# willSapgreen/stereo-vision

Hardware: AMD Instinct MI355X
Metric: stereo pairs/sec (ELAS 1242x375, ROBOTICS, D1+D2+LR) (higher is better)
Workload: dtype u8

## Files before the change

### stereo-vision_amd/csrc/elas_engine.cpp

```cpp
#include <hip/hip_runtime.h>
#include <stdio.h>
#include <string.h>

#include <atomic>
#include <chrono>
#include <condition_variable>
#include <deque>
#include <functional>
#include <algorithm>
#include <map>
#include <memory>
#include <mutex>
#include <string>
#include <thread>
#include <vector>

#include "hip_guard.h"
#include "svh_internal.h"

namespace svh {

static thread_local int t_device = 0;

#define HIP_TRY(kind, expr) SVH_HIP_TRY(nullptr, kind, expr)
// ... 85 lines not shown
    size_t prior_cap = 0;
    size_t ntri_max = 0;
    std::vector<HostPrior> hp;
    std::vector<int32_t> P;
    StageDev stg{};
    bool stage_ok = false;
    hipEvent_t stage_ev = nullptr;
    bool resident = false;
    bool force_host = false;
    float P_key[5] = {-1, -1, -1, -1, -1};
    static constexpr int kHist = 4;
    int32_t hist_sup[kHist] = {}, hist_tri[kHist] = {};
    int hist_n = 0, hist_at = 0;
    int32_t hist_g = 0;
    svh_elas_params hist_p{};
    PhaseBSize sized{};
    size_t o_P = 0, o_sup = 0, o_tri = 0;

    void release() {
        if (!stream) return;
        (void)hipSetDevice(device);
        static_cast<LaneBufs&>(*this) = LaneBufs();
        stage_ok = false; stg = StageDev{};
        P_key[0] = -1;
        hist_n = 0;
        W = H = 0;
    }

    void destroy() {
        if (!stream) return;
        (void)hipSetDevice(device);
        release();
        for (hipEvent_t* e : {&wait_ev, &match_ev, &copy_ev, &stage_ev})
            if (*e) {
                (void)hipEventDestroy(*e);
                *e = nullptr;
            }
        for (hipEvent_t e : prof.ev) (void)hipEventDestroy(e);
        prof.ev.clear();
        prof.names.clear();
        if (copy_stream) (void)hipStreamDestroy(copy_stream);
        (void)hipStreamDestroy(stream);
        copy_stream = stream = nullptr;
    }

    int ensure(const svh_elas_params& p, int32_t w, int32_t h, int32_t g) {
        if (!stream) {
            HIP_TRY(none, hipSetDevice(device));
            HIP_TRY(none, hipStreamCreateWithFlags(&stream, hipStreamNonBlocking));
        }
        const int32_t st = p.candidate_stepsize + (p.subsampling ? p.candidate_stepsize % 2 : 0);
        if (w == W && h == H && p.disp_max == disp_max && st == step && p.grid_size == grid_size &&
            p.subsampling == sub && g <= gcap)
            return SVH_OK;
        hipStream_t keep = stream;
        release();
        stream = keep;
        d = make_dims(p, w, h);
        const size_t N = (size_t)w * h, DN = (size_t)d.DW * d.DH, G2 = (size_t)2 * g;
        LANE_GROW(img, G2 * N);
        LANE_GROW(desc, G2 * N * 16);
        LANE_GROW(owner, G2 * N * sizeof(int32_t));
        HIP_TRY(copy, hipMemset(owner, 0, G2 * N * sizeof(int32_t)));
        owner_hi = svh::env("SVH_TEST_OWNER_HI") ? atoll(svh::env("SVH_TEST_OWNER_HI")) : 0;
        LANE_GROW(Draw, G2 * DN * sizeof(float));
        LANE_GROW(D, G2 * DN * sizeof(float));
        LANE_GROW(tmp, G2 * DN * sizeof(float));
        LANE_GROW(labels, G2 * DN * sizeof(int32_t));
        LANE_GROW(counts, G2 * DN * sizeof(int32_t));
        LANE_GROW(seg_nroots, G2 * (size_t)((d.DW + 63) / 64) * ((d.DH + 15) / 16) * sizeof(int32_t));
        const size_t nc = (size_t)d.Wc * d.Hc;
        LANE_GROW(dcan, g * nc * sizeof(int16_t));
        LANE_GROW(h_dcan, g * nc * sizeof(int16_t));
        LANE_GROW(h_img, G2 * N);
        const size_t nsup = nc + 6;
        ntri_max = 2 * nsup + 8;
        prior_cap = sizeof(GroupHdr) + (size_t)(p.disp_max + 1) * sizeof(int32_t) + 512 +
                    (size_t)g * (nsup * 3 + 2 * ntri_max * 3) * sizeof(int32_t);
        LANE_GROW(prior_dev, prior_cap);
        LANE_GROW(h_prior, prior_cap);
        LANE_GROW(raster, G2 * ntri_max * sizeof(TriRaster));
        LANE_GROW(planes, G2 * ntri_max * 6 * sizeof(float));
        const size_t gw_bytes = G2 * d.gw * d.gh * d.gwords * sizeof(uint32_t);
        LANE_GROW(seed, gw_bytes);
        LANE_GROW(mask, gw_bytes);
        if (d.gwords <= 8) LANE_GROW(lists, G2 * d.gw * d.gh * 32 * sizeof(uint16_t));
        hp.resize(g);
        o_P = (sizeof(GroupHdr) + 63) & ~(size_t)63;
        o_sup = (o_P + (size_t)(p.disp_max + 1) * sizeof(int32_t) + 63) & ~(size_t)63;
        o_tri = (o_sup + (size_t)g * nsup * 3 * sizeof(int32_t) + 63) & ~(size_t)63;
        if (stage_device_ok(p, d) && o_tri + (size_t)g * 2 * ntri_max * 3 * sizeof(int32_t) <= prior_cap) {
            const size_t cap = std::min<size_t>(nsup, 65535), rec = 2 * cap + 2, S2 = (size_t)2 * g;
            size_t off = 0;
            auto take = [&](size_t bytes) { size_t at = off; off = (off + bytes + 255) & ~(size_t)255; return at; };
            const size_t a_sup = take((size_t)g * 3 * cap * 4), a_cnt = take(sizeof(StageCounts));
            const size_t a_ids = take(S2 * 4 * rec * 4), a_xys = take(S2 * 4 * rec * 4), a_nbr = take(S2 * 4 * rec * 4);
            size_t a_arr[11];
            for (int k = 0; k < 11; k++) a_arr[k] = take(S2 * cap * 4);
            const size_t a_fl = take(S2 * 2 * cap * 4), a_fr = take(S2 * 2 * cap * 4);
            const size_t a_wl = take((size_t)g * 3 * nc * 4), a_cw = take((size_t)g * (nc / 4 + 1) * 4);
            LANE_GROW(stage_blob, off);
            HIP_TRY(copy, hipMemset(stage_blob, 0, off));
            LANE_GROW(h_counts, sizeof(StageCounts));
            uint8_t* b = stage_blob;
            stg.dcan = dcan;
            stg.sup_raw = reinterpret_cast<int32_t*>(b + a_sup);
            stg.counts = reinterpret_cast<StageCounts*>(b + a_cnt);
            stg.ids = reinterpret_cast<int32_t*>(b + a_ids);
            stg.xys = reinterpret_cast<int32_t*>(b + a_xys);
            stg.nbr = reinterpret_cast<uint32_t*>(b + a_nbr);
            int32_t** ia[6] = {&stg.pxy, &stg.buck, &stg.buck2, &stg.byx, &stg.order, &stg.oxy};
            uint32_t** ua[4] = {&stg.lx, &stg.ly, &stg.tmp, &stg.P};
            for (int k = 0; k < 6; k++) *ia[k] = reinterpret_cast<int32_t*>(b + a_arr[k]);
            for (int k = 0; k < 4; k++) *ua[k] = reinterpret_cast<uint32_t*>(b + a_arr[6 + k]);
            stg.dmap = reinterpret_cast<int32_t*>(b + a_arr[10]);
            stg.fl = reinterpret_cast<uint32_t*>(b + a_fl);
            stg.fr = reinterpret_cast<uint32_t*>(b + a_fr);
            stg.wl = reinterpret_cast<int32_t*>(b + a_wl);
            stg.cntw = reinterpret_cast<uint32_t*>(b + a_cw);
            stg.sup_cap = (int32_t)cap;
            stg.rec_cap = (int32_t)rec;
            stage_ok = true;
        }
        HIP_TRY(wait, hipDeviceSynchronize());
        W = w; H = h; disp_max = p.disp_max; step = st; grid_size = p.grid_size; sub = p.subsampling;
        gcap = g;
        return SVH_OK;
    }
};

static std::atomic<int> g_wait_us{40};
static std::atomic<bool> g_hostprof{false};
static hipError_t lane_wait(Lane& L) {
    if (!L.poll_wait || g_wait_us <= 0) return hipStreamSynchronize(L.stream);
    if (!L.wait_ev) {
        hipError_t e = hipEventCreateWithFlags(&L.wait_ev, hipEventDisableTiming);
        if (e != hipSuccess) return e;
    }
    hipError_t e = hipEventRecord(L.wait_ev, L.stream);
    if (e != hipSuccess) return e;
    for (;;) {
        e = hipEventQuery(L.wait_ev);
        if (e != hipErrorNotReady) return e;
        std::this_thread::sleep_for(std::chrono::microseconds(g_wait_us.load(std::memory_order_relaxed)));
    }
}

struct Pool {
    std::mutex mu;
    std::condition_variable cv;
    std::vector<Lane*> lanes;
    std::vector<Lane*> free_list;
    int max_lanes = 4;
};

static std::mutex g_mu;

static std::map<int, Pool*>& g_pools = *new std::map<int, Pool*>();
static std::atomic<int> g_lanes{6};
static std::atomic<int> g_group{32};
static std::atomic<bool> g_group_set{false};
static std::atomic<int> g_stage_mode{-1};
static int stage_mode_from_env();
static void apply_config(const svh_config& c, int explicit_call) {
    if (explicit_call) {
        if (c.elas_workers > 0) svh_elas_set_lanes(c.elas_workers);
        if (c.elas_pairs_per_launch > 0) svh_elas_set_group(c.elas_pairs_per_launch);
// ... 405 lines not shown
                for (int k = 0; k < 2 && pinned; k++) {
                    hipPointerAttribute_t at;
                    pinned = hipPointerGetAttributes(&at, io.hI[k][j]) == hipSuccess && at.type == hipMemoryTypeHost;
                }
            (void)hipGetLastError();
            if (pinned) {
                static const bool strided_up = !(svh::env("SVH_H2D_STRIDED") && atoi(svh::env("SVH_H2D_STRIDED")) == 0);
                for (int k = 0; k < 2; k++)
                    for (int32_t j = 0; j < g;) {
                        uint8_t* dst = L.img + ((size_t)2 * j + k) * N;
                        if (io.pitch != W) {
                            HIP_TRY(copy, hipMemcpy2DAsync(dst, W, io.hI[k][j], io.pitch, W, H, hipMemcpyHostToDevice, s));
                            j++;
                            continue;
                        }
                        int32_t e = j + 1;
                        while (strided_up && e < g && io.hI[k][e] == io.hI[k][e - 1] + N) e++;
                        if (e - j > 1)
                            HIP_TRY(copy, hipMemcpy2DAsync(dst, 2 * N, io.hI[k][j], N, N, (size_t)(e - j), hipMemcpyHostToDevice, s));
                        else
                            HIP_TRY(copy, hipMemcpyAsync(dst, io.hI[k][j], N, hipMemcpyHostToDevice, s));
                        j = e;
                    }
            } else {
                for (int32_t j = 0; j < g; j++)
                    for (int k = 0; k < 2; k++) {
                        uint8_t* dst = L.h_img + ((size_t)2 * j + k) * N;
                        const uint8_t* src = io.hI[k][j];
                        if (io.pitch == W) memcpy(dst, src, N);
                        else
                            for (int32_t v = 0; v < H; v++) memcpy(dst + (size_t)v * W, src + (size_t)v * io.pitch, W);
                    }
                HIP_TRY(copy, hipMemcpyAsync(L.img, L.h_img, (size_t)2 * g * N, hipMemcpyHostToDevice, s));
            }
            img.I[0] = L.img; img.I[1] = L.img + N;
            img.stride = 2 * N; img.pitch = W;
        }
        {
            std::vector<int32_t> Pt;
            int32_t pr = 2;
            prior_table(p, Pt, &pr);
            int32_t absmax = 0;
            for (int32_t dd = 0; dd <= pr && dd < (int32_t)Pt.size(); dd++)
                absmax = std::max(absmax, (int32_t)std::min<int64_t>(std::llabs((long long)Pt[dd]), INT32_MAX));
            static const int fly_env = svh::env("SVH_DESC_FLY") ? atoi(svh::env("SVH_DESC_FLY")) : 1;
            L.desc_fly = (!tapping || fly_env == 2) && descriptors_on_the_fly(p, d, absmax, pr, L.lists != nullptr);
        }
        if (tapping && L.desc_fly) {
            launch_descriptor(cx, img, g, W, H, p.subsampling, L.desc, false);
            int rc2 = tap_dev(L, taps, SVH_ELAS_DESC1, L.desc.p, N * 16); if (rc2) return rc2;
            rc2 = tap_dev(L, taps, SVH_ELAS_DESC2, L.desc.p + N * 16, N * 16); if (rc2) return rc2;
            HIP_TRY(wait, hipStreamSynchronize(s));
        }
        launch_descriptor(cx, img, g, W, H, p.subsampling, L.desc, L.desc_fly);
        launch_support(cx, p, d, g, L.desc, L.dcan, L.desc_fly);
        const int sm = g_stage_mode.load();
        L.resident = !L.force_host && L.stage_ok &&
                     (sm == 1 || (sm < 0 && prefer_device && stage_device_preferred(p, d, prefer_device > 1)));
        if (L.resident && prefer_device) L.poll_wait = true;
        if (!L.resident || tapping)
            HIP_TRY(copy, hipMemcpyAsync(L.h_dcan, L.dcan, g * nc * sizeof(int16_t), hipMemcpyDeviceToHost, s));
        if (L.resident) {
            prior_table(p, L.P, &plane_radius);
            const float key[5] = {p.beta, p.gamma, p.sigma, p.sradius, (float)p.disp_max};
            if (memcmp(key, L.P_key, sizeof(key)) != 0) {
                memcpy(L.h_prior + L.o_P, L.P.data(), L.P.size() * sizeof(int32_t));
                HIP_TRY(copy, hipMemcpyAsync(L.prior_dev + L.o_P, L.h_prior + L.o_P, L.P.size() * sizeof(int32_t),
                                       hipMemcpyHostToDevice, s));
                HIP_TRY(wait, hipStreamSynchronize(s));
                memcpy(L.P_key, key, sizeof(key));
            }
            if (tapping) {
                HIP_TRY(wait, hipStreamSynchronize(s));
                if (!L.desc_fly) {
                    rc = tap_dev(L, taps, SVH_ELAS_DESC1, L.desc.p, N * 16); if (rc) return rc;
                    rc = tap_dev(L, taps, SVH_ELAS_DESC2, L.desc.p + N * 16, N * 16); if (rc) return rc;
                }
                tap_host(taps, SVH_ELAS_DCAN_RAW, L.h_dcan.p, nc);
            }
            const bool blits = svh::env("SVH_STAGE_BLITS") && atoi(svh::env("SVH_STAGE_BLITS")) != 0;
            launch_stage_device(cx, p, d, g, L.stg, reinterpret_cast<GroupHdr*>(L.prior_dev.p),
                                reinterpret_cast<int32_t*>(L.prior_dev + L.o_sup),
                                reinterpret_cast<int32_t*>(L.prior_dev + L.o_tri),
                                blits ? nullptr : L.seed.p, (size_t)2 * g * d.gw * d.gh * d.gwords,
                                blits ? nullptr : L.h_counts.p);
            if (!L.stage_ev) HIP_TRY(none, hipEventCreateWithFlags(&L.stage_ev, hipEventDisableTiming));
            if (blits) HIP_TRY(copy, hipMemcpyAsync(L.h_counts, L.stg.counts, sizeof(StageCounts), hipMemcpyDeviceToHost, s));
            HIP_TRY(none, hipEventRecord(L.stage_ev, s));
            if (tapping) {
                HIP_TRY(copy, hipMemcpyAsync(hdr, L.prior_dev, sizeof(GroupHdr), hipMemcpyDeviceToHost, s));
                HIP_TRY(wait, hipStreamSynchronize(s));
                if (hdr->active[0]) {
                    rc = tap_dev(L, taps, SVH_ELAS_SUPPORT, reinterpret_cast<int32_t*>(L.prior_dev + L.o_sup),
                                 (size_t)3 * hdr->total_sup); if (rc) return rc;
                    rc = tap_dev(L, taps, SVH_ELAS_TRI1, reinterpret_cast<int32_t*>(L.prior_dev + L.o_tri),
                                 (size_t)3 * hdr->tri_end[0]); if (rc) return rc;
                    rc = tap_dev(L, taps, SVH_ELAS_TRI2,
                                 reinterpret_cast<int32_t*>(L.prior_dev + L.o_tri) + (size_t)3 * hdr->tri_end[0],
                                 (size_t)3 * (hdr->tri_end[1] - hdr->tri_end[0])); if (rc) return rc;
                }
            }
            L.sized = PhaseBSize{};
            if (!tapping || hdr->active[0]) {
                const int32_t tri_bound = 2 * g * 2 * L.stg.sup_cap;
                int32_t hint_sup = 0, hint_tri = 0;
                const bool use_hist = !(svh::env("SVH_PHASEB_HISTORY") && atoi(svh::env("SVH_PHASEB_HISTORY")) == 0);
                if (use_hist && L.hist_n && L.hist_g == g && memcmp(&L.hist_p, &p, sizeof(p)) == 0)
                    for (int k = 0; k < L.hist_n; k++) {
                        hint_sup = std::max(hint_sup, L.hist_sup[k]);
                        hint_tri = std::max(hint_tri, L.hist_tri[k]);
                    }
                L.sized = phase_b_size(d, g, -1, -1, hint_sup, hint_tri);
                L.sized.seed_cleared = !blits;
                rc = enqueue_phase_b(L.o_P, L.o_sup, L.o_tri, -1, -1, tri_bound, L.sized);
                if (rc) return rc;
            }
        }
        HP_MARK(HP_ENQ_A);
    }
    if (!(mode & RG_HOST_B)) return SVH_OK;
    double t1 = t0, t2 = t0;
    if (L.resident) {
        if (!io.out_device) {
            HIP_TRY(wait, event_wait(L, L.stage_ev));
            HP_MARK(HP_WAIT);
            int32_t active[kMaxGroup];
            for (int32_t j = 0; j < g; j++) active[j] = active_of(j);
            rc = copy_out(active);
            if (rc) return rc;
        }
        if (g_hostprof) g_hp_pairs += g;
        HP_MARK(HP_ENQ_B);
        t1 = t2 = now_ms();
    } else {
    const bool warm = L.parallel_host && g == 1;
    if (warm) helpers_warm(3, 1500);
    struct WarmOff {
        bool on;
        ~WarmOff() { if (on) helpers_warm(0, 0); }
    } warm_off{warm};
    HIP_TRY(wait, lane_wait(L));
    HIP_TRY(launch, hipGetLastError());
    L.prof.collect();
    HP_MARK(HP_WAIT);
    if (g_hostprof) g_hp_pairs += g;
    t1 = now_ms();
    if (tapping) {
        if (!L.desc_fly) {
            rc = tap_dev(L, taps, SVH_ELAS_DESC1, L.desc.p, N * 16); if (rc) return rc;
            rc = tap_dev(L, taps, SVH_ELAS_DESC2, L.desc.p + N * 16, N * 16); if (rc) return rc;
        }
        tap_host(taps, SVH_ELAS_DCAN_RAW, L.h_dcan.p, nc);
    }

    memset(hdr, 0, sizeof(GroupHdr));
    hdr->npairs = g;
    int32_t total_sup = 0, total_tri = 0, nactive = 0;
    for (int32_t j = 0; j < g; j++) {
        HostPrior& hp = L.hp[j];
        support_from_candidates(p, d, L.h_dcan + j * nc, hp.support, false);
        HP_MARK(HP_FILTER);
        hdr->sup_off[j] = total_sup;
        status[j] = SVH_OK;
        if (hp.support.size() / 3 < 3) {
            printf("ERROR: Need at least 3 support points!\n");
            fflush(stdout);
            status[j] = SVH_ERR_FEW_SUPPORT;
// ... 834 lines not shown
```

### stereo-vision_amd/csrc/elas_kernels.hip

```cpp
#include <hip/hip_runtime.h>

#include <algorithm>
#include <cstdlib>

#include "dev_common.h"
#include "prior_core.h"
#include "svh_internal.h"

namespace svh {

namespace {

constexpr int kWave = 64;

template <int kCtrl, int kRowMask>
__device__ __forceinline__ uint32_t dpp_min_step(uint32_t v) {
    const uint32_t o =
        (uint32_t)__builtin_amdgcn_update_dpp((int)0xFFFFFFFFu, (int)v, kCtrl, kRowMask, 0xF, false);
    return o < v ? o : v;
}

__device__ __forceinline__ uint32_t wave_min_u32(uint32_t v) {
    v = dpp_min_step<0xB1, 0xF>(v);
    v = dpp_min_step<0x4E, 0xF>(v);
// ... 557 lines not shown
            const int x0 = rgt ? xr0 : xl0, x1 = rgt ? xr1 : xl1, w = rgt ? wrs : wls;
            uint4* dst = (rgt ? sR : sL) + row * w - x0;
#pragma unroll
            for (int i = 0; i < 4; i++)
                if (x + i >= x0 && x + i <= x1) dst[x + i] = o[i];
        }
        for (int task = (int)threadIdx.x; task < nr + kSB; task += kST) {
            if (task < nr) {
                const int x = ar0 + 4 * task;
                uint4 o[4];
                fly_desc4_off(pl1, imstride + (uint32_t)v * fpitch + 8u + (uint32_t)x, fpitch, vplane, o);
                if (x == 0 || x + 4 > P.W - 3) {
#pragma unroll
                    for (int i = 0; i < 4; i++)
                        if (x + i < 3 || x + i >= P.W - 3) o[i] = make_uint4(0, 0, 0, 0);
                }
#pragma unroll
                for (int i = 0; i < 4; i++)
                    if (x + i >= xr0 && x + i <= xr1) s_texR[x + i - xr0] = (uint16_t)texture16(o[i]);
            } else {
                const int c = task - nr, u = (uc0 + c) * P.step;
                s_texL[c] = (uint16_t)(c < ncand && u < P.W ? texture16(fly_desc1(pl1, P.W, P.H, u, v)) : 0u);
            }
        }
    } else {
    stage_slots<6>(s_strip, 2 * (wls + wrs), (int)threadIdx.x, kST, [&](int i) {
        const bool rgt = i >= 2 * wls;
        const int j = rgt ? i - 2 * wls : i, w = rgt ? wrs : wls, wreal = rgt ? wr : wl;
        const int row = j >= w, xx = j - row * w, x = xx < wreal ? xx : wreal - 1;
        return (rgt ? d2 : d1)[(size_t)(v + (row ? 2 : -2)) * P.W + (rgt ? xr0 : xl0) + x];
    });
    }
    __syncthreads();
    const StripView L = {sL, xl0, wls}, R = {sR, xr0, wrs};
    constexpr int kNW = kST / kWave, kPerRound = 4 * kNW;
    static_assert(kSB % kPerRound == 0 && kSB <= 256, "whole rounds; candidate indices fit a byte");
    const int grp = lane >> 4;
    const int gl = lane & 15;
    __shared__ int16_t s_fwd[kSB];
    __shared__ uint8_t s_todo[kSB];
    __shared__ int s_ntodo;
#pragma unroll
    for (int rep = 0; rep < kSB / kPerRound; rep++) {
        const int c = rep * kPerRound + wave + grp * kNW;
        if (rep * kPerRound >= ncand) break;
        const bool have = c < ncand;
        const int uc = uc0 + (have ? c : 0), u = uc * P.step;
        const bool in = have && uc > 0 && u >= 5 && u <= P.W - 6;
        const int t1 = !in ? 0 : kFly ? (int)s_texL[c] : (int)texture16(d1[(size_t)v * P.W + u]);
        const int d = support_match_rows(L, R, t1, u, false, in, P, gl);
        if (gl == 0 && c < kSB) s_fwd[c] = (int16_t)(have ? d : -1);
    }
    __syncthreads();
    if (wave == 0) {
        int base = 0;
#pragma unroll
        for (int c0 = 0; c0 < kSB; c0 += kWave) {
            const int c = c0 + lane;
            const int mine = c < ncand ? (int)s_fwd[c] : -1;
            const uint64_t mask = __builtin_amdgcn_ballot_w64(mine >= 0);
            if (mine >= 0) s_todo[base + __builtin_popcountll(mask & ((1ull << lane) - 1))] = (uint8_t)c;
            base += __builtin_popcountll(mask);
            if (c < ncand && mine < 0) dcan[c] = (int16_t)((uc0 + c) > 0 ? -1 : 0);
        }
        if (lane == 0) s_ntodo = base;
    }
    __syncthreads();
    const int ntodo = s_ntodo;
    for (int t0 = 4 * wave; t0 < ntodo; t0 += kPerRound) {
        const int t = t0 + grp;
        const bool have = t < ntodo;
        const int c = have ? (int)s_todo[t] : 0;
        const int d = have ? (int)s_fwd[c] : 0;
        const int uc = uc0 + c, u = uc * P.step;
        const int ub = have ? u - d : 5;
        const int t2 = !have ? 0 : kFly ? (int)s_texR[ub - xr0] : (int)texture16(d2[(size_t)v * P.W + ub]);
        const int dd = support_match_rows(R, L, t2, ub, true, have, P, gl);
        const int diff = d > dd ? d - dd : dd - d;
        const int out = (dd >= 0 && diff <= P.lr_threshold) ? d : -1;
        if (have && gl == 0) dcan[c] = (int16_t)out;
    }
}

__global__ __launch_bounds__(256) void k_prior(GroupDev G, int total_tri_arg) {
    const int total_tri = total_tri_arg >= 0 ? total_tri_arg : G.hdr->total_tri;
    for (int gid = blockIdx.x * 256 + threadIdx.x; (gid - (int)threadIdx.x) < 2 * total_tri; gid += gridDim.x * 256) {
    const int T = gid >> 1, rs = gid & 1;
    const bool live = T < total_tri;
    const int Tc = live ? T : 0;
    int first;
    const int slot = tri_slot(G.hdr, Tc, &first);
    const int pair = slot >> 1, side = slot & 1;
    const int32_t* sup = G.support + 3 * (size_t)G.hdr->sup_off[pair];
    const int32_t* c = G.tri + 3 * (size_t)Tc;
    int32_t su[3], sv[3], sd[3];
#pragma unroll
    for (int k = 0; k < 3; k++) {
        const int32_t* s = sup + 3 * c[k];
        su[k] = s[0];
        sv[k] = s[1];
        sd[k] = s[2];
    }
    float mine[3];
    {
        double A[3][3], B[3];
#pragma unroll
        for (int r = 0; r < 3; r++) {
            A[r][0] = (double)(rs ? su[r] - sd[r] : su[r]);
            A[r][1] = (double)sv[r];
            A[r][2] = 1.0;
            B[r] = (double)sd[r];
        }
        if (prior::solve3(A, B)) {
            mine[0] = (float)B[0];
            mine[1] = (float)B[1];
            mine[2] = (float)B[2];
        } else {
            mine[0] = mine[1] = mine[2] = 0.f;
        }
    }
    float pl[6];
#pragma unroll
    for (int k = 0; k < 3; k++) {
        const float other = __shfl_xor(mine[k], 1);
        pl[k] = rs ? other : mine[k];
        pl[3 + k] = rs ? mine[k] : other;
    }
    if (!live || rs) continue;
#pragma unroll
    for (int k = 0; k < 6; k++) G.planes[6 * (size_t)T + k] = pl[k];

    float tu[3], tv[3];
#pragma unroll
    for (int k = 0; k < 3; k++) {
        tu[k] = side ? (float)(su[k] - sd[k]) : (float)su[k];
        tv[k] = (float)sv[k];
    }
#pragma unroll
    for (int j = 0; j < 3; j++)
#pragma unroll
        for (int k = 0; k < j; k++)
            if (tu[k] > tu[j]) {
                float a = tu[j]; tu[j] = tu[k]; tu[k] = a;
                float b = tv[j]; tv[j] = tv[k]; tv[k] = b;
            }
    TriRaster r;
    const float Au = tu[0], Av = tv[0], Bu = tu[1], Bv = tv[1], Cu = tu[2], Cv = tv[2];
    r.uA = (int32_t)Au;
    r.uB = (int32_t)Bu;
    r.uC = (int32_t)Cu;
    float ABa = 0.f, ACa = 0.f, BCa = 0.f;
    if (r.uA != r.uB) ABa = __fdiv_rn(__fsub_rn(Av, Bv), __fsub_rn(Au, Bu));
    if (r.uA != r.uC) ACa = __fdiv_rn(__fsub_rn(Av, Cv), __fsub_rn(Au, Cu));
    if (r.uB != r.uC) BCa = __fdiv_rn(__fsub_rn(Bv, Cv), __fsub_rn(Bu, Cu));
    r.ABa = ABa;
    r.ACa = ACa;
    r.BCa = BCa;
    r.ABb = __fsub_rn(Av, __fmul_rn(ABa, Au));
    r.ACb = __fsub_rn(Av, __fmul_rn(ACa, Au));
    r.BCb = __fsub_rn(Bv, __fmul_rn(BCa, Bu));
    const float pa = side ? pl[3] : pl[0];
    const float pd = side ? pl[0] : pl[3];
    r.pa = pa;
    r.pb = side ? pl[4] : pl[1];
    r.pc = side ? pl[5] : pl[2];
    r.valid = ((double)fabsf(pa) < 0.7 && (double)fabsf(pd) < 0.7) ? 1 : 0;
    r.slot = slot;
    r.first = first;
    r.pad_[0] = 0;
    G.raster[T] = r;
    }
}

__global__ __launch_bounds__(256) void k_grid_seed(GroupDev G, int total_sup_arg, int gw, int gh,
                                                   int gwords, int grid_size, int disp_max) {
    const int total_sup = total_sup_arg >= 0 ? total_sup_arg : G.hdr->total_sup;
    for (int S = blockIdx.x * 256 + threadIdx.x; S < total_sup; S += gridDim.x * 256) {
    int pair = 0;
    while (pair < G.hdr->npairs - 1 && S >= G.hdr->sup_off[pair + 1]) pair++;
    const int32_t* s = G.support + 3 * (size_t)S;
    const int xc = s[0], yc = s[1], dc = s[2];
    const int y = (int)floorf(__fdiv_rn((float)yc, (float)grid_size));
    const int xl = (int)floorf((float)(xc / grid_size));
    const int xr = (int)floorf(__fdiv_rn((float)(xc - dc), (float)grid_size));
    const int lo = dc - 1 > 0 ? dc - 1 : 0, hi = dc + 1 < disp_max ? dc + 1 : disp_max;
    const size_t cells = (size_t)gw * gh;
#pragma unroll
    for (int side = 0; side < 2; side++) {
        const int x = side ? xr : xl;
        if (x < 0 || x >= gw || y < 0 || y >= gh) continue;
        uint32_t* cell = G.seed + (((size_t)(2 * pair + side) * cells) + (size_t)y * gw + x) * gwords;
        for (int dd = lo; dd <= hi; dd++) atomicOr(&cell[dd >> 5], 1u << (dd & 31));
    }
    }
}

__global__ __launch_bounds__(256) void k_grid_dilate(GroupDev G, int slots, int gw, int gh,
                                                     int gwords) {
    const int i = blockIdx.x * 256 + threadIdx.x;
    const int cells = gw * gh;
    const int per = cells * gwords;
    if (i >= slots * per) return;
    const int z = i / per, rem = i - z * per;
    const int c = rem / gwords, w = rem - c * gwords;
    uint32_t o = 0;
    if (c >= gw + 1 && c <= cells - gw - 2) {
        const uint32_t* base = G.seed + (size_t)z * per + w;
        const int nb[9] = {-gw - 1, -gw, -gw + 1, -1, 0, 1, gw - 1, gw, gw + 1};
#pragma unroll
        for (int k = 0; k < 9; k++) o |= base[(size_t)(c + nb[k]) * gwords];
    }
    G.mask[i] = o;
}

__global__ __launch_bounds__(256) void k_grid_list(GroupDev G, int ncells, int gwords) {
    const int lane = threadIdx.x & 63;
    const int cell = __builtin_amdgcn_readfirstlane((int)((blockIdx.x * 256 + threadIdx.x) >> 6));
    if (cell >= ncells) return;
    const uint32_t* bits = G.mask + (size_t)cell * gwords;
    const uint32_t wq = lane < gwords ? bits[lane] : 0u;
    uint16_t* rec = G.lists + (size_t)cell * 32;
    int n = 0, last = 0;
#pragma unroll
    for (int q = 0; q < 4; q++) {
        const uint64_t m = (uint64_t)(uint32_t)__builtin_amdgcn_readlane((int)wq, 2 * q) |
                           ((uint64_t)(uint32_t)__builtin_amdgcn_readlane((int)wq, 2 * q + 1) << 32);
        if ((m >> lane) & 1) {
            const int idx = n + (int)__builtin_amdgcn_mbcnt_hi((uint32_t)(m >> 32), __builtin_amdgcn_mbcnt_lo((uint32_t)m, 0));
            if (idx < 28) rec[idx] = (uint16_t)((64 * q + lane) * 16);
        }
        if (m) last = 64 * q + 63 - __builtin_clzll(m);
        n += __builtin_popcountll(m);
    }
    if (lane < 31 && lane >= n) rec[lane] = (uint16_t)(last * 16);
    if (lane == 31) rec[31] = (uint16_t)n;
    if (lane >= 28 && lane < 31 && lane < n) rec[lane] = (uint16_t)(last * 16);
}

template <bool kFix>
__global__ __launch_bounds__(256) void k_owner(GroupDev G, int total_tri_arg, int W, int H, int sub, int fix_all) {
    const int total_tri = total_tri_arg >= 0 ? total_tri_arg : G.hdr->total_tri;
    const int lane = threadIdx.x & 63;
    const int need = (((total_tri + 3) >> 2) + 7) >> 3, have = (int)(gridDim.x >> 3);
    const int per_xcd = need < have ? need : have;
    if ((int)(blockIdx.x >> 3) >= per_xcd) return;
    const int bid = (int)(blockIdx.x & 7) * per_xcd + (int)(blockIdx.x >> 3);
    for (int T = __builtin_amdgcn_readfirstlane((int)((bid * 256 + threadIdx.x) >> 6)); T < total_tri;
         T += per_xcd * 32) {
    const TriRaster tr = G.raster[T];
    const int slot = tr.slot, first = tr.first;
    const int t = G.owner_base + 1 + (T - first);
    int32_t* owner = G.owner + (size_t)slot * W * H;
    const int cl = lane & 15, rp = lane >> 4;
    {
        const int ulo = tr.uA > 2 ? tr.uA : 2, uhi = tr.uC < W - 2 ? tr.uC : W - 2;
        for (int u = ulo + cl; u < uhi; u += 16) {
            if (sub && (u & 1)) continue;
            const bool second = u >= tr.uB;
            const float ea = second ? tr.BCa : tr.ABa, eb = second ? tr.BCb : tr.ABb;
            const float fu = (float)u;
            const int v1 = f2u2i(__fadd_rn(__fmul_rn(tr.ACa, fu), tr.ACb));
            const int v2 = f2u2i(__fadd_rn(__fmul_rn(ea, fu), eb));
            int va = v1 < v2 ? v1 : v2, vb = v1 < v2 ? v2 : v1;
            va = va > 0 ? va : 0;
            vb = vb < H ? vb : H;
            if (kFix && !fix_all) {
                const int v = rp < 2 ? va + rp : vb - 4 + rp;
                const bool mine = v >= va && v < vb && (rp < 2 || v >= va + 2);
                if (mine && !(sub && (v & 1))) {
                    int32_t* px = &owner[(size_t)v * W + u];
                    if (*px < t) atomicMax(px, t);
                }
            } else {
                for (int v = va + rp; v < vb; v += 4) {
                    if (sub && (v & 1)) continue;
                    int32_t* px = &owner[(size_t)v * W + u];
                    if (kFix) {
                        if (*px < t) atomicMax(px, t);
                    } else {
                        *px = t;
                    }
                }
            }
        }
    }
    }
}

struct MatchParams {
    int W, H, DW, DH, gw, gh, gwords, grid_size, sub;
    int disp_max, match_texture, plane_radius, npairs;
    uint32_t grid_magic;
};

template <bool kLds>
__global__ __launch_bounds__(kLds ? 512 : 256) void k_match(GroupDev G, MatchParams P) {
    extern __shared__ uint4 s_row[];
    __shared__ int s_P[64];
    const int z = blockIdx.z, pair = z >> 1, side = z & 1;
    if (!G.hdr->active[pair]) return;
    const int y = kLds ? blockIdx.y : blockIdx.y * 4 + threadIdx.y;
    {
        const int tl = kLds ? (int)threadIdx.x : (int)(threadIdx.y * 64 + threadIdx.x);
        if (tl < 64) s_P[tl] = tl <= P.disp_max ? G.P[tl] : 0;
    }
    const size_t N = (size_t)P.W * P.H;
    const int mul = P.sub ? 2 : 1;
    const int v = y * mul;
    int line = v < P.H - 3 ? v : P.H - 3;
    line = line > 2 ? line : 2;
    const uint4* oth_line =
        reinterpret_cast<const uint4*>(G.desc + (size_t)(z ^ 1) * N * 16) + (size_t)line * P.W;
    const int s0 = 0;
    if (kLds)
        for (int i = threadIdx.x; i < P.W; i += blockDim.x) s_row[i] = oth_line[i];
    __syncthreads();
    for (int x = kLds ? (int)threadIdx.x : (int)(blockIdx.x * 64 + threadIdx.x); x < P.DW;
         x += kLds ? (int)blockDim.x : P.DW) {
    if (y >= P.DH) return;
    const int u = x * mul;
    float out = -10.f;
    const int tri0 = z ? G.hdr->tri_end[z - 1] : 0;
    const int t = G.owner[(size_t)z * N + (size_t)v * P.W + u] - G.owner_base - 1;
    if (t >= 0 && u >= 2 && u < P.W - 2) {
        const uint4* own_line =
            reinterpret_cast<const uint4*>(G.desc + (size_t)z * N * 16) + (size_t)line * P.W;
        const uint4 own = own_line[u];
        if ((int)texture16(own) >= P.match_texture) {
            const float4 pl = *reinterpret_cast<const float4*>(G.raster + tri0 + t);
            const float pa = pl.x, pb = pl.y, pc = pl.z;
            const int valid = __float_as_int(pl.w);
            const int d_plane = (int)__fadd_rn(
                __fadd_rn(__fmul_rn(pa, (float)u), __fmul_rn(pb, (float)v)), pc);
            int dlo = d_plane - P.plane_radius;
            dlo = dlo > 0 ? dlo : 0;
            int dhi = d_plane + P.plane_radius;
            dhi = dhi < P.disp_max ? dhi : P.disp_max;
            const int cell = (v / P.grid_size) * P.gw + u / P.grid_size;
            const uint32_t* bits = G.mask + ((size_t)z * P.gw * P.gh + cell) * P.gwords;
            int min_val = 10000, min_d = -1;
            uint32_t wbuf[8];
            const bool fast8 = P.gwords == 8;
            if (fast8) {
                const uint4 lo4 = reinterpret_cast<const uint4*>(bits)[0];
                const uint4 hi4 = reinterpret_cast<const uint4*>(bits)[1];
                wbuf[0] = lo4.x; wbuf[1] = lo4.y; wbuf[2] = lo4.z; wbuf[3] = lo4.w;
                wbuf[4] = hi4.x; wbuf[5] = hi4.y; wbuf[6] = hi4.z; wbuf[7] = hi4.w;
            }
            for (int w = 0; w < P.gwords; w++) {
                uint32_t b;
                if (fast8) {
                    b = wbuf[0];
#pragma unroll
                    for (int q = 1; q < 8; q++) b = (w == q) ? wbuf[q] : b;
                } else {
                    b = bits[w];
                }
                while (b) {
                    const int dc = w * 32 + __builtin_ctz(b);
                    b &= b - 1;
                    if (dc < dlo || dc > dhi) {
                        const int uw = side ? u + dc : u - dc;
                        if (uw < 2 || uw >= P.W - 2) continue;
                        const uint4 o = kLds ? s_row[uw - s0] : oth_line[uw];
                        const int val = (int)sad16(own, o);
                        if (val < min_val) {
                            min_val = val;
                            min_d = dc;
// ... 1365 lines not shown
        if (p) p->end();
    }
};

#define LAUNCH(name, kernel, grid, block, ...)                                                  \
    do {                                                                                        \
        Timed timed_(cx, name);                                                                 \
        hipLaunchKernelGGL(kernel, grid, block, 0, (hipStream_t)cx.stream, __VA_ARGS__);        \
    } while (0)

}

void launch_descriptor(const LaunchCtx& cx, const DevImages& img, int32_t g, int32_t W, int32_t H,
                       int32_t half, uint8_t* desc, bool fly) {
    if (fly) {
        const int strips = (W + 4 * 62 - 1) / (4 * 62);
        const int cols = 4 * ((W + 4 * strips - 1) / (4 * strips));
        const int segs = (H + SP_ROWS - 1) / SP_ROWS, nwaves = strips * segs;
        LAUNCH("k_descriptor", k_sobel_planes, dim3((nwaves + 3) / 4, 2 * g), dim3(256), img, W, H, strips, cols,
               nwaves, desc);
        return;
    }
    constexpr int rows = 26, chunk = 16;
    static_assert((rows + 6) % chunk == 0, "the walk is a whole number of load chunks");
    const int strips = (W + DS_COLS - 1) / DS_COLS, segs = (H + rows - 1) / rows, nwaves = strips * segs;
    LAUNCH("k_descriptor", (k_descriptor_stream<rows, chunk>), dim3((nwaves + 3) / 4, 2 * g), dim3(256), img, W, H,
           half, strips, nwaves, desc);
}

static int support_strip(const svh_elas_params& p, const Dims& d, size_t* lds_out) {
    static const int sb_env = svh::env("SVH_SUPPORT_SB") ? atoi(svh::env("SVH_SUPPORT_SB")) : 64;
    constexpr size_t kSupportStatic = 512;
    auto strip_lds = [&](int sb) {
        const int span = (sb - 1) * d.step;
        const size_t wl = (size_t)std::min(d.W, span + 2 * p.disp_max + 5);
        const size_t wr = (size_t)std::min(d.W, span + p.disp_max + 5);
        return 2 * (size_t)(support_stride((int)wl) + support_stride((int)wr)) * sizeof(uint4);
    };
    int sb = sb_env == 32 ? 32 : 64;
    if (sb == 64 && strip_lds(64) + 2 * (size_t)d.W + 16 + kSupportStatic > 64 * 1024) sb = 32;
    const size_t lds = strip_lds(sb) + 2 * (size_t)std::min(d.W, (sb - 1) * d.step + p.disp_max + 5) + 16;
    if (lds_out) *lds_out = lds;
    return lds + kSupportStatic <= 64 * 1024 ? sb : 0;
}

void launch_support(const LaunchCtx& cx, const svh_elas_params& p, const Dims& d, int32_t g,
                    const uint8_t* desc, int16_t* dcan, bool fly) {
    SupportParams P;
    P.W = d.W; P.H = d.H; P.Wc = d.Wc; P.Hc = d.Hc; P.step = d.step; P.npairs = g;
    P.disp_min = p.disp_min; P.disp_max = p.disp_max;
    P.support_texture = p.support_texture; P.lr_threshold = p.lr_threshold;
    P.support_threshold = p.support_threshold;
    size_t lds = 0;
    const int sb = support_strip(p, d, &lds);
    if (sb) {
        Timed timed_(cx, "k_support");
        const int chunks = (d.Wc + sb - 1) / sb;
        const dim3 grid((unsigned)(((d.Hc * g + 7) / 8) * 8 * chunks), 1, 1);
        hipStream_t st = (hipStream_t)cx.stream;
        if (sb == 32 && fly) hipLaunchKernelGGL((k_support_lds<32, 512, true>), grid, dim3(512), lds, st, desc, dcan, P);
        else if (sb == 32) hipLaunchKernelGGL((k_support_lds<32, 512, false>), grid, dim3(512), lds, st, desc, dcan, P);
        else if (fly) hipLaunchKernelGGL((k_support_lds<64, 512, true>), grid, dim3(512), lds, st, desc, dcan, P);
        else hipLaunchKernelGGL((k_support_lds<64, 512, false>), grid, dim3(512), lds, st, desc, dcan, P);
    } else {
        const int cands = d.Wc * d.Hc;
        LAUNCH("k_support", k_support, dim3((cands + 3) / 4, g), dim3(256), desc, dcan, P);
    }
}

PhaseBSize phase_b_size(const Dims& d, int32_t g, int32_t total_sup, int32_t total_tri, int32_t hint_sup, int32_t hint_tri) {
    const int sup_bound = std::max(256, g * d.Wc * d.Hc / 6), tri_bound = 4 * sup_bound;
    PhaseBSize z;
    z.from_history = total_tri < 0 && total_sup < 0 && hint_sup > 0 && hint_tri > 0;
    z.ns = total_sup >= 0 ? total_sup : z.from_history ? std::min(sup_bound, hint_sup + hint_sup / 8 + 1) : sup_bound;
    z.nt = total_tri >= 0 ? total_tri : z.from_history ? std::min(tri_bound, hint_tri + hint_tri / 8 + 1) : tri_bound;
    z.seed_cleared = false;
    return z;
}

void launch_prior(const LaunchCtx& cx, const svh_elas_params& p, const Dims& d, int32_t g,
                  int32_t total_sup, int32_t total_tri, const GroupDev& G, const PhaseBSize& size) {
    hipStream_t s = (hipStream_t)cx.stream;
    const int cells = d.gw * d.gh;
    const size_t words = (size_t)2 * g * cells * d.gwords;
    if (!size.seed_cleared) (void)hipMemsetAsync(G.seed, 0, words * sizeof(uint32_t), s);
    const int nt = size.nt, ns = size.ns;
    if (nt > 0) LAUNCH("k_prior", k_prior, dim3((2 * nt + 255) / 256), dim3(256), G, total_tri);
    if (ns > 0)
        LAUNCH("k_grid_seed", k_grid_seed, dim3((ns + 255) / 256), dim3(256), G, total_sup,
               d.gw, d.gh, d.gwords, p.grid_size, p.disp_max);
    LAUNCH("k_grid_dilate", k_grid_dilate, dim3((unsigned)((words + 255) / 256)), dim3(256), G,
           2 * g, d.gw, d.gh, d.gwords);
    if (d.gwords <= 8 && G.lists)
        LAUNCH("k_grid_list", k_grid_list, dim3((unsigned)((2 * g * cells + 3) / 4)), dim3(256), G, 2 * g * cells,
               d.gwords);
}

void launch_owner(const LaunchCtx& cx, const svh_elas_params& p, const Dims& d, int32_t g,
                  int32_t total_tri, const GroupDev& G, const PhaseBSize& size) {
    if (total_tri == 0) return;
    const int nt = size.nt;
    const bool wide = (double)d.H * ((double)d.W + 2.0 * p.disp_max) > 4194304.0;
    const int fix_all = svh::env("SVH_OWNER_FIX_ALL") ? atoi(svh::env("SVH_OWNER_FIX_ALL")) : (wide ? 1 : 0);
    const dim3 go(xcd_blocks((nt + 3) / 4));
    LAUNCH("k_owner", k_owner<false>, go, dim3(256), G, total_tri, d.W, d.H,
           p.subsampling, 0);
    LAUNCH("k_owner_fix", k_owner<true>, go, dim3(256), G, total_tri, d.W, d.H,
           p.subsampling, fix_all);
}

static bool match_list_usable(const svh_elas_params& p, const Dims& d, int32_t prior_absmax, int32_t plane_radius,
                              bool have_lists, MatchList* Qout, size_t* lds_out) {
    static const bool ordered = svh::env("SVH_MATCH_ORDERED") != nullptr;
    const bool keyed_ok = !ordered && prior_absmax < (1 << 19) && p.disp_max < 512 && plane_radius <= 15 &&
                          d.W < 65536 && p.grid_size > 1;
    static const bool list_off = svh::env("SVH_MATCH_LIST") && atoi(svh::env("SVH_MATCH_LIST")) == 0;
    static const bool list_sub = !(svh::env("SVH_MATCH_LIST_SUB") && atoi(svh::env("SVH_MATCH_LIST_SUB")) == 0);
    if (!(keyed_ok && !list_off && (!p.subsampling || list_sub) && d.gwords <= 8 && have_lists && prior_absmax < 28000 &&
          d.DW <= 8 * 256))
        return false;
    MatchList Q;
    Q.Wr = (d.W + 7) / 8 * 8;
    Q.Ws = ((d.W + 3) & ~3) + 2;
    static const bool wide768 = !(svh::env("SVH_MATCH_WIDE768") && atoi(svh::env("SVH_MATCH_WIDE768")) == 0);
    int iters = (d.DW + 255) / 256;
    Q.half = std::min(256, ((d.DW + iters - 1) / iters + 63) / 64 * 64);
    if (iters > 5 && wide768 && d.DW <= 5 * 384) {
        iters = (d.DW + 383) / 384;
        Q.half = std::min(384, ((d.DW + iters - 1) / iters + 63) / 64 * 64);
    }
    Q.kIters = iters <= 5 ? 5 : 8;
    static const bool xcd_rows = !(svh::env("SVH_MATCH_XCD") && atoi(svh::env("SVH_MATCH_XCD")) == 0);
    Q.xcd = xcd_rows ? 1 : 0;
    const size_t ldsl = (size_t)2 * Q.Ws * sizeof(uint4) + (size_t)2 * d.gw * ML_CAP * sizeof(uint16_t) +
                        (size_t)2 * Q.Wr * sizeof(int16_t);
    constexpr size_t kListStatic = 256;
    bool ok = ldsl + kListStatic <= 160 * 1024;
    if (ok && ldsl + kListStatic > 64 * 1024) {
        ok = hipFuncSetAttribute((const void*)k_match_list<true, 5>, hipFuncAttributeMaxDynamicSharedMemorySize,
                                 160 * 1024 - (int)kListStatic) == hipSuccess &&
             hipFuncSetAttribute((const void*)k_match_list<false, 5>, hipFuncAttributeMaxDynamicSharedMemorySize,
                                 160 * 1024 - (int)kListStatic) == hipSuccess &&
             hipFuncSetAttribute((const void*)k_match_list<true, 8>, hipFuncAttributeMaxDynamicSharedMemorySize,
                                 160 * 1024 - (int)kListStatic) == hipSuccess &&
             hipFuncSetAttribute((const void*)k_match_list<false, 8>, hipFuncAttributeMaxDynamicSharedMemorySize,
                                 160 * 1024 - (int)kListStatic) == hipSuccess;
        if (!ok) (void)hipGetLastError();
    }
    if (Qout) *Qout = Q;
    if (lds_out) *lds_out = ldsl;
    return ok;
}

static bool match_keyed_usable(const svh_elas_params& p, const Dims& d, int32_t prior_absmax, int32_t plane_radius,
                               bool with_lr, size_t* lds2_out) {
    static const bool ordered = svh::env("SVH_MATCH_ORDERED") != nullptr;
    const bool keyed_ok = !ordered && prior_absmax < (1 << 19) && p.disp_max < 512 && plane_radius <= 15 &&
                          d.W < 65536 && p.grid_size > 1;
    const size_t lds = (size_t)d.W * sizeof(uint4);
    const size_t lds2 = 2 * lds + (with_lr ? (size_t)2 * d.DW * sizeof(float) : 0);
    if (lds2_out) *lds2_out = lds2;
    constexpr size_t keyed_lds_max = 96 * 1024;
    constexpr size_t kStaticLds = 64 * sizeof(int);
    bool use_keyed = keyed_ok && lds2 + kStaticLds <= keyed_lds_max;
    if (use_keyed && lds2 + kStaticLds > 64 * 1024) {
        use_keyed = hipFuncSetAttribute((const void*)k_match_keyed<true>, hipFuncAttributeMaxDynamicSharedMemorySize,
                                        (int)keyed_lds_max) == hipSuccess &&
                    hipFuncSetAttribute((const void*)k_match_keyed<false>, hipFuncAttributeMaxDynamicSharedMemorySize,
                                        (int)keyed_lds_max) == hipSuccess;
        if (!use_keyed) (void)hipGetLastError();
    }
    return use_keyed;
}

bool descriptors_on_the_fly(const svh_elas_params& p, const Dims& d, int32_t prior_absmax, int32_t plane_radius,
                            bool have_lists) {
    static const bool off = svh::env("SVH_DESC_FLY") && atoi(svh::env("SVH_DESC_FLY")) == 0;
    static const bool keyed_fly = !(svh::env("SVH_DESC_FLY_KEYED") && atoi(svh::env("SVH_DESC_FLY_KEYED")) == 0);
    if (off || d.W < 8 || support_strip(p, d, nullptr) == 0) return false;
    if (match_list_usable(p, d, prior_absmax, plane_radius, have_lists, nullptr, nullptr)) return true;
    return keyed_fly && match_keyed_usable(p, d, prior_absmax, plane_radius, true, nullptr);
}

bool launch_match(const LaunchCtx& cx, const svh_elas_params& p, const Dims& d, int32_t g,
                  const GroupDev& G, const DevMaps* lr_out, bool write_raw, const char** error) {
    if (error) *error = nullptr;
    MatchParams P;
    P.W = d.W; P.H = d.H; P.DW = d.DW; P.DH = d.DH; P.gw = d.gw; P.gh = d.gh; P.gwords = d.gwords;
    P.grid_size = p.grid_size; P.sub = p.subsampling; P.disp_max = p.disp_max;
    P.match_texture = p.match_texture; P.plane_radius = G.plane_radius;
    P.grid_magic = (uint32_t)(0x100000000ull / (uint64_t)p.grid_size) + 1u;
// ... 430 lines not shown
```

### stereo-vision_amd/csrc/svh_internal.h

```cpp
#ifndef SVH_INTERNAL_H
#define SVH_INTERNAL_H

#include <stddef.h>
#include <stdint.h>

#include <functional>
#include <vector>

#include "../../include/svh.h"
#include "svh_config.h"

namespace svh {

struct Dims {
    int32_t W, H;
    int32_t DW, DH;
    int32_t step;
    int32_t Wc, Hc;
    int32_t gw, gh;
    int32_t gwords;
};
Dims make_dims(const svh_elas_params& p, int32_t W, int32_t H);

constexpr int kMaxGroup = 32;
// ... 41 lines not shown
    int32_t ntri[2 * kMaxGroup];
    int32_t flags[kMaxGroup];
    int64_t dbg[32];
    int32_t dt_m[2 * kMaxGroup];
    int32_t dt_depth[2 * kMaxGroup];
};
enum { STG_DUP = 1,
       STG_OVERFLOW = 2,
       STG_FEW = 4 };
struct StageDev {
    int16_t* dcan;
    int32_t* sup_raw;
    StageCounts* counts;
    int32_t* ids;
    int32_t* xys;
    uint32_t* nbr;
    int32_t *pxy, *buck, *buck2, *byx, *order, *oxy;
    int32_t* dmap;
    uint32_t *lx, *ly, *tmp, *P;
    uint32_t *fl, *fr;
    int32_t* wl;
    uint32_t* cntw;
    int32_t sup_cap, rec_cap;
};
struct LaunchCtx;
bool stage_device_ok(const svh_elas_params& p, const Dims& d);
bool stage_device_preferred(const svh_elas_params& p, const Dims& d, bool deep_batch = false);

struct Profiler {
    virtual void begin(const char* kernel) = 0;
    virtual void end() = 0;
    virtual ~Profiler() {}
};
struct LaunchCtx {
    void* stream;
    Profiler* prof;
    bool latency = false;
};

struct DevImages {
    const uint8_t* I[2];
    size_t stride;
    int32_t pitch;
};
struct DevMaps {
    float* D[2];
    size_t stride[2];
};

struct GroupDev {
    const GroupHdr* hdr;
    const int32_t* support;
    const int32_t* tri;
    const int32_t* P;
    TriRaster* raster;
    float* planes;
    uint32_t* seed;
    uint32_t* mask;
    uint16_t* lists;
    const uint8_t* desc;
    int32_t* owner;
    float* Draw;
    int32_t plane_radius;
    int32_t owner_base;
    int32_t prior_absmax;
    int32_t desc_fly;
};

void launch_stage_device(const LaunchCtx& cx, const svh_elas_params& p, const Dims& d, int32_t g,
                         const StageDev& S, GroupHdr* hdr, int32_t* support, int32_t* tri,
                         uint32_t* seed, size_t seed_words, StageCounts* h_counts);

void launch_descriptor(const LaunchCtx& cx, const DevImages& img, int32_t g, int32_t W, int32_t H,
                       int32_t half, uint8_t* desc, bool fly);
bool descriptors_on_the_fly(const svh_elas_params& p, const Dims& d, int32_t prior_absmax, int32_t plane_radius,
                            bool have_lists);
void launch_support(const LaunchCtx& cx, const svh_elas_params& p, const Dims& d, int32_t g,
                    const uint8_t* desc, int16_t* dcan, bool fly);
struct PhaseBSize {
    int32_t ns, nt;
    bool from_history;
    bool seed_cleared;
};
PhaseBSize phase_b_size(const Dims& d, int32_t g, int32_t total_sup, int32_t total_tri, int32_t hint_sup, int32_t hint_tri);
void launch_prior(const LaunchCtx& cx, const svh_elas_params& p, const Dims& d, int32_t g,
                  int32_t total_sup, int32_t total_tri, const GroupDev& G, const PhaseBSize& size);
void launch_owner(const LaunchCtx& cx, const svh_elas_params& p, const Dims& d, int32_t g,
                  int32_t total_tri, const GroupDev& G, const PhaseBSize& size);
bool launch_match(const LaunchCtx& cx, const svh_elas_params& p, const Dims& d, int32_t g,
                  const GroupDev& G, const DevMaps* lr_out, bool write_raw, const char** error);
void launch_lr(const LaunchCtx& cx, const svh_elas_params& p, const Dims& d, int32_t g,
               const GroupDev& G, const DevMaps& out);
struct PostScratch {
    float* tmp;
    int32_t* labels;
    int32_t* counts;
    int32_t* nroots;
};
bool post_tiles_ok(const svh_elas_params& p);
void launch_gap_mean_tiles(const LaunchCtx& cx, const svh_elas_params& p, const Dims& d, int32_t g,
                           int32_t nside, const GroupDev& G, const DevMaps& out, const PostScratch& S);
void launch_segments(const LaunchCtx& cx, const svh_elas_params& p, const Dims& d, int32_t g,
                     int32_t nside, const GroupDev& G, const DevMaps& out, const PostScratch& s, bool mask = true);
void launch_gap(const LaunchCtx& cx, const svh_elas_params& p, const Dims& d, int32_t g,
                int32_t nside, const GroupDev& G, const DevMaps& out, const PostScratch& s);
void launch_adaptive_mean(const LaunchCtx& cx, const svh_elas_params& p, const Dims& d, int32_t g,
                          int32_t nside, const GroupDev& G, const DevMaps& out, const PostScratch& s);
void launch_median(const LaunchCtx& cx, const Dims& d, int32_t g, int32_t nside, const GroupDev& G,
                   const DevMaps& out, const PostScratch& s);
void launch_segments_label(const LaunchCtx& cx, const svh_elas_params& p, const Dims& d, int32_t g,
                           int32_t nside, const GroupDev& G, const DevMaps& in, const PostScratch& s);

}
#endif
```

Before: 34230.

## Replace full owner fix pass with corner-only pass guarded by per-slot validity flags

k_prior now checks whether the float edge rasterization is consistent with the integer vertices and sets a per-slot flag when it is not, and k_owner flags slots whose edge spans look inverted. The owner fix pass becomes a lighter k_owner_corner kernel that touches only the corner columns of each triangle unless its slot is flagged, in which case it walks all columns. The flags sit at the tail of the seed buffer, which is grown and cleared to hold them. This cuts the second full per-triangle column walk, at the cost of extra checks in k_prior and k_owner, and correctness now depends on the flag heuristics catching every case.

```diff
diff --git a/stereo-vision_amd/csrc/elas_engine.cpp b/stereo-vision_amd/csrc/elas_engine.cpp
--- a/stereo-vision_amd/csrc/elas_engine.cpp
+++ b/stereo-vision_amd/csrc/elas_engine.cpp
@@ -191,7 +191,7 @@
         LANE_GROW(raster, G2 * ntri_max * sizeof(TriRaster));
         LANE_GROW(planes, G2 * ntri_max * 6 * sizeof(float));
         const size_t gw_bytes = G2 * d.gw * d.gh * d.gwords * sizeof(uint32_t);
-        LANE_GROW(seed, gw_bytes);
+        LANE_GROW(seed, gw_bytes + G2 * sizeof(uint32_t));
         LANE_GROW(mask, gw_bytes);
         if (d.gwords <= 8) LANE_GROW(lists, G2 * d.gw * d.gh * 32 * sizeof(uint16_t));
         hp.resize(g);
@@ -763,7 +763,7 @@
             launch_stage_device(cx, p, d, g, L.stg, reinterpret_cast<GroupHdr*>(L.prior_dev.p),
                                 reinterpret_cast<int32_t*>(L.prior_dev + L.o_sup),
                                 reinterpret_cast<int32_t*>(L.prior_dev + L.o_tri),
-                                blits ? nullptr : L.seed.p, (size_t)2 * g * d.gw * d.gh * d.gwords,
+                                blits ? nullptr : L.seed.p, seed_words_with_flags(d, g),
                                 blits ? nullptr : L.h_counts.p);
             if (!L.stage_ev) HIP_TRY(none, hipEventCreateWithFlags(&L.stage_ev, hipEventDisableTiming));
             if (blits) HIP_TRY(copy, hipMemcpyAsync(L.h_counts, L.stg.counts, sizeof(StageCounts), hipMemcpyDeviceToHost, s));
diff --git a/stereo-vision_amd/csrc/elas_kernels.hip b/stereo-vision_amd/csrc/elas_kernels.hip
--- a/stereo-vision_amd/csrc/elas_kernels.hip
+++ b/stereo-vision_amd/csrc/elas_kernels.hip
@@ -663,7 +663,7 @@
     }
 }
 
-__global__ __launch_bounds__(256) void k_prior(GroupDev G, int total_tri_arg) {
+__global__ __launch_bounds__(256) void k_prior(GroupDev G, int total_tri_arg, uint32_t* __restrict__ oflag) {
     const int total_tri = total_tri_arg >= 0 ? total_tri_arg : G.hdr->total_tri;
     for (int gid = blockIdx.x * 256 + threadIdx.x; (gid - (int)threadIdx.x) < 2 * total_tri; gid += gridDim.x * 256) {
     const int T = gid >> 1, rs = gid & 1;
@@ -748,7 +748,31 @@
     r.valid = ((double)fabsf(pa) < 0.7 && (double)fabsf(pd) < 0.7) ? 1 : 0;
     r.slot = slot;
     r.first = first;
-    r.pad_[0] = 0;
+    {
+        const long long cr = (long long)(r.uB - r.uA) * (long long)((int)Cv - (int)Av) -
+                             (long long)((int)Bv - (int)Av) * (long long)(r.uC - r.uA);
+        const int sgn = cr > 0 ? 1 : cr < 0 ? -1 : 0;
+        r.pad_[0] = sgn;
+        bool bad = false;
+        if (r.uA < r.uC) {
+            const int iAv = (int)Av, iBv = (int)Bv;
+            const int kAC = f2u2i(__fadd_rn(__fmul_rn(r.ACa, Au), r.ACb));
+            bad = kAC != iAv && kAC != iAv - 1;
+            if (r.uA < r.uB) {
+                const int kAB = f2u2i(__fadd_rn(__fmul_rn(r.ABa, Au), r.ABb));
+                bad = bad || (kAB != iAv && kAB != iAv - 1);
+            }
+            if (r.uB < r.uC) {
+                const int kBC = f2u2i(__fadd_rn(__fmul_rn(r.BCa, Bu), r.BCb));
+                bad = bad || (kBC != iBv && kBC != iBv - 1);
+                if (r.uA < r.uB) {
+                    const int kACb = f2u2i(__fadd_rn(__fmul_rn(r.ACa, Bu), r.ACb));
+                    bad = bad || (sgn > 0 ? kACb < iBv : sgn < 0 ? kACb >= iBv : true);
+                }
+            }
+        }
+        if (bad) oflag[slot] = 1u;
+    }
     G.raster[T] = r;
     }
 }
@@ -819,7 +843,8 @@
 }
 
 template <bool kFix>
-__global__ __launch_bounds__(256) void k_owner(GroupDev G, int total_tri_arg, int W, int H, int sub, int fix_all) {
+__global__ __launch_bounds__(256) void k_owner(GroupDev G, int total_tri_arg, int W, int H, int sub, int fix_all,
+                                               uint32_t* __restrict__ oflag) {
     const int total_tri = total_tri_arg >= 0 ? total_tri_arg : G.hdr->total_tri;
     const int lane = threadIdx.x & 63;
     const int need = (((total_tri + 3) >> 2) + 7) >> 3, have = (int)(gridDim.x >> 3);
@@ -833,6 +858,7 @@
     const int t = G.owner_base + 1 + (T - first);
     int32_t* owner = G.owner + (size_t)slot * W * H;
     const int cl = lane & 15, rp = lane >> 4;
+    bool inverted = !kFix && fix_all != 0;
     {
         const int ulo = tr.uA > 2 ? tr.uA : 2, uhi = tr.uC < W - 2 ? tr.uC : W - 2;
         for (int u = ulo + cl; u < uhi; u += 16) {
@@ -845,6 +871,7 @@
             int va = v1 < v2 ? v1 : v2, vb = v1 < v2 ? v2 : v1;
             va = va > 0 ? va : 0;
             vb = vb < H ? vb : H;
+            if (!kFix) inverted = inverted || (u != tr.uA && (v1 < v2 ? tr.pad_[0] >= 0 : (v1 > v2 && tr.pad_[0] <= 0)));
             if (kFix && !fix_all) {
                 const int v = rp < 2 ? va + rp : vb - 4 + rp;
                 const bool mine = v >= va && v < vb && (rp < 2 || v >= va + 2);
@@ -865,6 +892,43 @@
             }
         }
     }
+    if (!kFix && inverted) oflag[slot] = 1u;
+    }
+}
+
+__global__ __launch_bounds__(256) void k_owner_corner(GroupDev G, int total_tri_arg, int W, int H, int sub,
+                                                      const uint32_t* __restrict__ oflag) {
+    const int total_tri = total_tri_arg >= 0 ? total_tri_arg : G.hdr->total_tri;
+    const int need = (((total_tri + 31) >> 5) + 7) >> 3, have = (int)(gridDim.x >> 3);
+    const int per_xcd = need < have ? need : have;
+    if ((int)(blockIdx.x >> 3) >= per_xcd) return;
+    const int bid = (int)(blockIdx.x & 7) * per_xcd + (int)(blockIdx.x >> 3);
+    const int col = (threadIdx.x >> 2) & 1, rp = threadIdx.x & 3;
+    for (int T = bid * 32 + (int)(threadIdx.x >> 3); T < total_tri; T += per_xcd * 256) {
+        const TriRaster tr = G.raster[T];
+        const int t = G.owner_base + 1 + (T - tr.first);
+        int32_t* owner = G.owner + (size_t)tr.slot * W * H;
+        const int ulo = tr.uA > 2 ? tr.uA : 2, uhi = tr.uC < W - 2 ? tr.uC : W - 2;
+        const bool walk = oflag[tr.slot] != 0;
+        int u = walk ? ulo + col : col ? tr.uB : tr.uA;
+        const int uend = walk ? uhi : (col && tr.uB == tr.uA) || u < ulo ? u : (u + 1 < uhi ? u + 1 : uhi);
+        for (; u < uend; u += 2) {
+            if (sub && (u & 1)) continue;
+            const bool second = u >= tr.uB;
+            const float ea = second ? tr.BCa : tr.ABa, eb = second ? tr.BCb : tr.ABb;
+            const float fu = (float)u;
+            const int v1 = f2u2i(__fadd_rn(__fmul_rn(tr.ACa, fu), tr.ACb));
+            const int v2 = f2u2i(__fadd_rn(__fmul_rn(ea, fu), eb));
+            int va = v1 < v2 ? v1 : v2, vb = v1 < v2 ? v2 : v1;
+            va = va > 0 ? va : 0;
+            vb = vb < H ? vb : H;
+            const int v = rp < 2 ? va + rp : vb - 4 + rp;
+            const bool mine = v >= va && v < vb && (rp < 2 || v >= va + 2);
+            if (mine && !(sub && (v & 1))) {
+                int32_t* px = &owner[(size_t)v * W + u];
+                if (*px < t) atomicMax(px, t);
+            }
+        }
     }
 }
 
@@ -2396,10 +2460,10 @@
                   int32_t total_sup, int32_t total_tri, const GroupDev& G, const PhaseBSize& size) {
     hipStream_t s = (hipStream_t)cx.stream;
     const int cells = d.gw * d.gh;
-    const size_t words = (size_t)2 * g * cells * d.gwords;
-    if (!size.seed_cleared) (void)hipMemsetAsync(G.seed, 0, words * sizeof(uint32_t), s);
+    const size_t words = seed_words(d, g);
+    if (!size.seed_cleared) (void)hipMemsetAsync(G.seed, 0, seed_words_with_flags(d, g) * sizeof(uint32_t), s);
     const int nt = size.nt, ns = size.ns;
-    if (nt > 0) LAUNCH("k_prior", k_prior, dim3((2 * nt + 255) / 256), dim3(256), G, total_tri);
+    if (nt > 0) LAUNCH("k_prior", k_prior, dim3((2 * nt + 255) / 256), dim3(256), G, total_tri, G.seed + words);
     if (ns > 0)
         LAUNCH("k_grid_seed", k_grid_seed, dim3((ns + 255) / 256), dim3(256), G, total_sup,
                d.gw, d.gh, d.gwords, p.grid_size, p.disp_max);
@@ -2416,11 +2480,17 @@
     const int nt = size.nt;
     const bool wide = (double)d.H * ((double)d.W + 2.0 * p.disp_max) > 4194304.0;
     const int fix_all = svh::env("SVH_OWNER_FIX_ALL") ? atoi(svh::env("SVH_OWNER_FIX_ALL")) : (wide ? 1 : 0);
+    const int force_walk = svh::env("SVH_OWNER_FORCE_WALK") && atoi(svh::env("SVH_OWNER_FORCE_WALK")) != 0 ? 1 : 0;
+    uint32_t* oflag = G.seed + seed_words(d, g);
     const dim3 go(xcd_blocks((nt + 3) / 4));
     LAUNCH("k_owner", k_owner<false>, go, dim3(256), G, total_tri, d.W, d.H,
-           p.subsampling, 0);
-    LAUNCH("k_owner_fix", k_owner<true>, go, dim3(256), G, total_tri, d.W, d.H,
-           p.subsampling, fix_all);
+           p.subsampling, force_walk, oflag);
+    if (fix_all == 0)
+        LAUNCH("k_owner_fix", k_owner_corner, dim3(xcd_blocks((nt + 31) / 32)), dim3(256), G, total_tri, d.W, d.H,
+               p.subsampling, oflag);
+    else
+        LAUNCH("k_owner_fix", k_owner<true>, go, dim3(256), G, total_tri, d.W, d.H,
+               p.subsampling, fix_all == 1 ? 1 : 0, oflag);
 }
 
 static bool match_list_usable(const svh_elas_params& p, const Dims& d, int32_t prior_absmax, int32_t plane_radius,
diff --git a/stereo-vision_amd/csrc/svh_internal.h b/stereo-vision_amd/csrc/svh_internal.h
--- a/stereo-vision_amd/csrc/svh_internal.h
+++ b/stereo-vision_amd/csrc/svh_internal.h
@@ -147,6 +147,8 @@
     bool from_history;
     bool seed_cleared;
 };
+inline size_t seed_words(const Dims& d, int32_t g) { return (size_t)2 * g * d.gw * d.gh * d.gwords; }
+inline size_t seed_words_with_flags(const Dims& d, int32_t g) { return seed_words(d, g) + (size_t)2 * g; }
 PhaseBSize phase_b_size(const Dims& d, int32_t g, int32_t total_sup, int32_t total_tri, int32_t hint_sup, int32_t hint_tri);
 void launch_prior(const LaunchCtx& cx, const svh_elas_params& p, const Dims& d, int32_t g,
                   int32_t total_sup, int32_t total_tri, const GroupDev& G, const PhaseBSize& size);
```

Measured after the change: 35540, median of 6. +3.8%, better.
